# jenkinsm13/julia-spira

Measured on AMD Instinct MI355X. Metric: Msamples/sec at 1920x1080 spp=64 depth=8; fraction of HBM roofline, higher is better.
Workload: dtype f64

## Files before the change

julia-spira_amd/csrc/spira_device.h:

```cpp
#pragma once
#include <hip/hip_runtime.h>
#include <stdint.h>
#include <type_traits>
#include "spira_fastdiv.h"

namespace spira {

__device__ __forceinline__ float sqrt_rn(float x) { return __builtin_sqrtf(x); }
__device__ __forceinline__ double sqrt_rn(double x) { return __builtin_sqrt(x); }

constexpr int kBlock = 256;
#ifndef SPIRA_WAVES_F32
#define SPIRA_WAVES_F32 5
#endif
#ifndef SPIRA_WAVES_F64
#define SPIRA_WAVES_F64 4
#endif
#define SPIRA_WAVES_PER_SIMD(T) (sizeof(T) == 8 ? SPIRA_WAVES_F64 : SPIRA_WAVES_F32)
constexpr uint32_t kMaxTries = 64;

template <class T> struct Vec { T x, y, z; };

template <class T> __device__ __forceinline__ Vec<T> mk(T x, T y, T z) { Vec<T> r; r.x = x; r.y = y; r.z = z; return r; }
template <class T> __device__ __forceinline__ Vec<T> operator+(Vec<T> a, Vec<T> b) { return mk<T>(a.x + b.x, a.y + b.y, a.z + b.z); }
// ... 1143 lines not shown
        }
        wave_lds_sync();
#pragma unroll
        for (int r = 0; r < R; ++r) {
            const bool alive = pend[r].kind != kDead;
            const unsigned long long m = __ballot(alive);
            if (alive) {
                Vec<T> rnd = mk<T>(0, 0, 0);
                if (pend[r].kind != kMirror) { const Pack4<T> w = s_rnd[ent[r]]; rnd = mk<T>(w.x, w.y, w.z); }
                const Vec<T> nd = segment_back<T>(o[r], pend[r], rnd);
                const uint32_t dst = region + fill + __popcll(m & lt_mask);
                Pack4<T> A, B; Pack2<T> C;
                A.x = o[r].x; A.y = o[r].y; A.z = o[r].z; A.w = nd.x;
                B.x = nd.y; B.y = nd.z; B.z = beta[r].x; B.w = beta[r].y;
                C.x = beta[r].z; C.y = Bits<T>::from_u32(q[r]);
                a.qout.A[dst] = A; a.qout.B[dst] = B; a.qout.C[dst] = C;
            }
            fill += (uint32_t)__popcll(m);
        }
        wave_lds_sync();
    }
    for (int sft = 32; sft > 0; sft >>= 1) { n_rmw += __shfl_down(n_rmw, sft); n_seg += __shfl_down(n_seg, sft); n_store += __shfl_down(n_store, sft); }
    if (lane == 0) {
        if (scatter) a.cnt_out[wid] = fill;
        a.blk_stats[4 * wid] = n_seg;
        a.blk_stats[4 * wid + 1] = n_rmw;
        a.blk_stats[4 * wid + 2] = n_store;
        a.blk_stats[4 * wid + 3] = FIRST ? 0u : n_seg;
    }
}

template <class T> struct PathArgs {
    SceneGlobal<T> scene;
    RenderConst<T> rc;
    RayQueue<T> q[2];
    uint32_t *qref[2];
    uint2 *qkey[2];
    uint32_t cam_consts;
    Pack3<T> *L;
    uint32_t *blk_stats;
    uint32_t cap;
    uint32_t pass;
    uint32_t n_first;
    uint32_t dense_pct;
    Pack4<T> *mesh_list;
    uint32_t mesh_min_batch;
    uint32_t refill_free;
    uint32_t mesh_mode;
    uint32_t *mesh_count;
    uint32_t resume_k, resume_nw;
    uint32_t *redo;
    uint32_t redo_only;
    Stats *stats;
};

__device__ __forceinline__ float pack_qref(uint32_t q, uint32_t, float) { return __uint_as_float(q); }
__device__ __forceinline__ double pack_qref(uint32_t q, uint32_t ref, double) { return __longlong_as_double((long long)((unsigned long long)q | ((unsigned long long)ref << 32))); }
__device__ __forceinline__ uint32_t unpack_q(float w) { return __float_as_uint(w); }
__device__ __forceinline__ uint32_t unpack_q(double w) { return (uint32_t)(unsigned long long)__double_as_longlong(w); }
__device__ __forceinline__ uint32_t unpack_ref(double w) { return (uint32_t)((unsigned long long)__double_as_longlong(w) >> 32); }

#ifdef SPIRA_MESH_STATS
__device__ unsigned long long g_mesh_dbg[32];
#define MESH_STAT(...) __VA_ARGS__
#else
#define MESH_STAT(...)
#endif

#ifndef SPIRA_CARRY_KEY
#define SPIRA_CARRY_KEY 1
#endif
#ifndef SPIRA_WAVES_B_F32
#define SPIRA_WAVES_B_F32 4
#endif
#ifndef SPIRA_WAVES_B_F64
#define SPIRA_WAVES_B_F64 SPIRA_WAVES_F64
#endif
#ifndef SPIRA_WAVES_PATH_F32
#define SPIRA_WAVES_PATH_F32 6
#endif
template <class T, int R, bool BVH, bool EXT, bool SPEC, int MODE = 0, bool TRI = true>
__global__ __launch_bounds__(kBlock, MODE == 2 ? (sizeof(T) == 8 ? SPIRA_WAVES_B_F64 : SPIRA_WAVES_B_F32) : (sizeof(T) == 4 ? SPIRA_WAVES_PATH_F32 : SPIRA_WAVES_F64)) void k_path(const PathArgs<T> a) {
    extern __shared__ __attribute__((aligned(32))) unsigned char lds_raw[];
    constexpr uint32_t WPB = kBlock / 64, SUB = 64 * R;
    constexpr bool kRefArray = sizeof(T) == 4;
    constexpr bool kCarry = SPIRA_CARRY_KEY && !BVH && !EXT;
    constexpr uint32_t kStageShift = 25, kRefMask = (1u << kStageShift) - 1u;
    const uint32_t lane = threadIdx.x & 63, wave = threadIdx.x >> 6;
    const uint32_t NW = gridDim.x * WPB, wid = blockIdx.x * WPB + wave;
    const RenderConst<T> &rc = a.rc;
    using Pol = typename std::conditional<SPEC, SpecDiv, ExactDiv>::type;
    Pol pol;
    if (!SPEC && a.redo_only) {
        uint32_t any = 0;
        for (uint32_t w = 0; w < WPB; ++w) any |= a.redo[blockIdx.x * WPB + w];
        if (!any) return;
    }
    T *cam_lds = reinterpret_cast<T *>(lds_raw + scene_lds_bytes<T>(a.scene.n_spheres, a.scene.n_materials, a.scene.n_triangles) + WPB * SUB * sizeof(Pack4<T>));
    if (threadIdx.x < 12) {
        const Vec<T> *cv = threadIdx.x < 3 ? &rc.cam_origin : (threadIdx.x < 6 ? &rc.cam_llc : (threadIdx.x < 9 ? &rc.cam_hor : &rc.cam_ver));
        const uint32_t cc = threadIdx.x % 3;
        cam_lds[threadIdx.x] = cc == 0 ? cv->x : (cc == 1 ? cv->y : cv->z);
    }
    Pack4<T> *cam_sph = reinterpret_cast<Pack4<T> *>(reinterpret_cast<unsigned char *>(cam_lds) + 128);
    constexpr bool kCam = !EXT;
    if (kCam && MODE != 2 && a.cam_consts)
        for (uint32_t i = threadIdx.x; i < a.scene.n_spheres; i += blockDim.x) {
            const T *sp = a.scene.spheres5 + 5 * (size_t)i;
            const Vec<T> oc = rc.cam_origin - mk<T>(sp[0], sp[1], sp[2]);
            Pack4<T> k; k.x = oc.x; k.y = oc.y; k.z = oc.z; k.w = dot(oc, oc) - sp[3] * sp[3];
            cam_sph[i] = k;
        }
    const SceneLds<T> sc = stage_scene<T>(a.scene, lds_raw);
    const PixelDiv<T> pix_div = pixel_divisors<T>(rc);
    if (!SPEC && a.redo_only) {
        if (!a.redo[wid]) return;
        if (lane == 0) atomicAdd(&a.stats->redone_waves, 1ull);
    }
    Pack4<T> *s_rnd = reinterpret_cast<Pack4<T> *>(lds_raw + scene_lds_bytes<T>(a.scene.n_spheres, a.scene.n_materials, a.scene.n_triangles)) + wave * SUB;
    constexpr uint32_t mesh_mode = BVH ? (uint32_t)MODE : 0u;
    const uint32_t kseg = mesh_mode == 2u ? a.resume_k : 1u;
    if (mesh_mode == 2u && wid * kseg >= a.resume_nw) return;
    const uint32_t region = wid * kseg * a.cap;
    const unsigned long long lt_mask = (1ull << lane) - 1ull;
    const uint32_t ref_base = sc.n_spheres + sc.n_triangles;
    const bool mixed = mesh_mode != 0u || rc.max_depth <= 128u;
    const uint32_t dense_pct = mixed ? a.dense_pct : 0u;
    const bool defer = mesh_mode != 0u || (BVH && mixed && a.mesh_list != nullptr);
    Pack4<T> *mlist = a.mesh_list + 3 * (size_t)region;
    uint32_t n_rmw = 0, n_store = 0, n_seg = 0, n_enq = 0, n_park = 0;
    uint32_t n_wtrips = 0, n_ltrips = 0;
    uint32_t n_in = 0;
    const uint32_t n_sub_first = (a.n_first + SUB - 1) / SUB;

    auto park = [&](uint32_t slot_i, const Vec<T> o_, const Vec<T> d_, const Vec<T> beta_, T closest_, uint32_t q_, int prim_, uint32_t stage_hit) {
        Pack4<T> A, B, C;
        A.x = o_.x; A.y = o_.y; A.z = o_.z; A.w = d_.x;
        B.x = d_.y; B.y = d_.z; B.z = beta_.x; B.w = beta_.y;
        C.x = beta_.z; C.y = closest_; C.z = Bits<T>::from_u32(q_); C.w = Bits<T>::from_u32((uint32_t)(prim_ + 1) | (stage_hit << kStageShift));
        mlist[3 * (size_t)slot_i] = A; mlist[3 * (size_t)slot_i + 1] = B; mlist[3 * (size_t)slot_i + 2] = C;
    };
    uint32_t mfill = 0;
    constexpr int kMaxSeg = 16;
    uint32_t pfx[kMaxSeg + 1];
    bool segmented = false;
    {
        uint32_t cnt = 0;
        if (mesh_mode == 2u && lane < kseg && wid * kseg + lane < a.resume_nw) cnt = a.mesh_count[wid * kseg + lane];
        pfx[0] = 0;
#pragma unroll
        for (int j = 0; j < kMaxSeg; ++j) pfx[j + 1] = pfx[j] + (uint32_t)__builtin_amdgcn_readlane((int)cnt, j);
        if (mesh_mode == 2u) { mfill = pfx[kMaxSeg]; segmented = true; }
    }
    const uint32_t first_sub = mesh_mode == 1u ? (wid % a.resume_k) * (NW / a.resume_k) + wid / a.resume_k : wid;
    MESH_STAT(unsigned long long dbg_t0 = __builtin_readcyclecounter(); unsigned long long dbg_sess = 0, dbg_walk = 0; uint32_t dbg_ns = 0, dbg_ws = 0, dbg_ls = 0, dbg_rf = 0, dbg_rays = 0, dbg_rounds = 0, dbg_ws1 = 0, dbg_ls1 = 0, dbg_h[4] = {0, 0, 0, 0};)
    for (uint32_t round = 0; ; ++round) {
        MESH_STAT(++dbg_rounds;)
        const bool first = mesh_mode != 2u && round == 0;
        const RayQueue<T> qin = a.q[(round + 1) & 1], qout = a.q[round & 1];
        const uint32_t *rin = a.qref[(round + 1) & 1];
        uint32_t *rout = a.qref[round & 1];
        const uint2 *kin = a.qkey[(round + 1) & 1];
        uint2 *kout = a.qkey[round & 1];
        const uint32_t limit = first ? a.n_first : n_in;
        const uint32_t n_sub = first ? n_sub_first : (n_in + SUB - 1) / SUB;
        uint32_t fill = 0;
        for (uint32_t sub = first ? first_sub : 0u; sub < n_sub; sub += first ? NW : 1u) {
            Vec<T> o[R], beta[R];
            Pending<T> pend[R];
            ExtState<T> ex[R];
            uint32_t q[R], ent[R], stg[R], ref[R];
            uint32_t ka[R], kb[R];
            bool valid[R];
#pragma unroll
            for (int r = 0; r < R; ++r) {
                const uint32_t idx = sub * SUB + r * 64 + lane;
                valid[r] = false; stg[r] = round; ref[r] = 0; q[r] = 0; ka[r] = 0; kb[r] = 0;
                pend[r].kind = kDead; pend[r].rough = 0; pend[r].v = mk<T>(0, 0, 0);
                o[r] = mk<T>(0, 0, 0); beta[r] = mk<T>(1, 1, 1);
                bool parked = false; T park_t = 0; int park_prim = -1;
                if (idx < limit) {
                    if (first) {
                        uint32_t pixel, sample, pi, pj;
                        Vec<T> d;
                        q[r] = idx;
                        path_of<T>(rc, idx, a.pass, pi, pj, pixel, sample);
                        if (kCarry) { ka[r] = mix32(rc.sA + pixel) ^ (sample << 8); kb[r] = mix32(rc.sB ^ pixel) + (sample << 8); }
                        camera_ray_lds<T>(rc, cam_lds, pix_div, pi, pj, pixel, sample, o[r], d, pol);
                        if (EXT) { ex[r].flags = rc.flags; if (rc.flags & kExtSpectral) beta[r] = ext_wavelength<T>(sc, rc.sA, rc.sB, pixel, sample, ex[r]); }
                        T t; uint32_t slot = 0;
                        int prim;
                        if (defer) {
                            if (kCam && a.cam_consts) closest_hit_local<T, Pol, TRI, true>(sc, o[r], d, (T)0.001, t, prim, pol, cam_sph);
                            else closest_hit_local<T, Pol, TRI>(sc, o[r], d, (T)0.001, t, prim, pol);
                            parked = mesh_box_hit<T>(sc, o[r], d, t);
                        } else if (kCam && !BVH && a.cam_consts) { closest_hit_local<T, Pol, TRI, true>(sc, o[r], d, (T)0.001, t, prim, pol, cam_sph); }
                        else prim = closest_hit<T, BVH, Pol, TRI>(sc, o[r], d, (T)0.001, t, slot, pol);
                        ++n_seg;
                        if (parked) { park_t = t; park_prim = prim; pend[r].v = d; }
                        else if (prim < 0) {
                            const Vec<T> c = sky_term_x<T, EXT>(d, beta[r], &ex[r]);
                            Pack3<T> l; l.x = c.x; l.y = c.y; l.z = c.z;
                            a.L[idx] = l;
                            ++n_store;
                        } else {
                            valid[r] = true;
                            o[r] = o[r] + d * t;
                            ref[r] = (BVH && prim >= (int)ref_base) ? ref_base + slot : (uint32_t)prim;
                            pend[r].v = d;
                        }
                    } else {
                        const Pack4<T> A = qin.A[region + idx], B = qin.B[region + idx];
                        const Pack2<T> C = qin.C[region + idx];
                        o[r] = mk<T>(A.x, A.y, A.z);
                        pend[r].v = mk<T>(A.w, B.x, B.y);
                        beta[r] = mk<T>(B.z, B.w, C.x);
                        q[r] = unpack_q(C.y);
                        uint32_t w;
                        if constexpr (kRefArray) w = rin[region + idx]; else w = unpack_ref(C.y);
                        if (mixed) { stg[r] = w >> kStageShift; ref[r] = w & kRefMask; } else ref[r] = w;
                        if (kCarry) { const uint2 k = kin[region + idx]; ka[r] = k.x; kb[r] = k.y; }
                        valid[r] = true;
                    }
                }
                if (defer && first) {
                    const unsigned long long mp = __ballot(parked);
                    if (parked) park(mfill + __popcll(mp & lt_mask), o[r], pend[r].v, beta[r], park_t, q[r], park_prim, 0u);
                    mfill += (uint32_t)__popcll(mp); n_park += (uint32_t)__popcll(mp);
                }
            }
            while (true) {
                uint32_t n_list = 0, n_valid = 0;
#pragma unroll
                for (int r = 0; r < R; ++r) {
                    bool want = false;
                    RngKey key;
                    const Vec<T> d = pend[r].v;
                    pend[r].kind = kDead;
                    if (valid[r]) {
                        uint32_t pixel = 0, sample = 0, pi, pj;
                        const bool scatter = stg[r] + 1 < rc.max_depth;
                        int prim = (int)ref[r]; uint32_t slot = 0;
                        if (BVH && ref[r] >= ref_base) { prim = (int)ref_base; slot = ref[r] - ref_base; }
                        const uint32_t qi = q[r] & 0x7FFFFFFFu;
                        const bool has_l = (q[r] >> 31) != 0;
                        if (EXT) {
                            path_of<T>(rc, qi, a.pass, pi, pj, pixel, sample);
                            ex[r].flags = rc.flags;
                            if (rc.flags & kExtSpectral) (void)ext_wavelength<T>(sc, rc.sA, rc.sB, pixel, sample, ex[r]);
                        }
                        Vec<T> contrib;
                        const bool has_contrib = shade_hit<T, BVH, EXT, Pol, TRI>(sc, o[r], d, prim, slot, beta[r], scatter, contrib, pend[r], &ex[r], pol);
                        if (has_contrib) {
                            Pack3<T> l; l.x = contrib.x; l.y = contrib.y; l.z = contrib.z;
                            if (has_l) { const Pack3<T> l0 = a.L[qi]; l.x = l0.x + contrib.x; l.y = l0.y + contrib.y; l.z = l0.z + contrib.z; ++n_rmw; }
                            else ++n_store;
// ... 293 lines not shown
                finished = false;
                const unsigned long long mf = __ballot(!walking);
                const uint32_t take = min((uint32_t)__popcll(mf), mfill - next);
                if (!walking && (uint32_t)__popcll(mf & lt_mask) < take) {
                    const uint32_t e = next + (uint32_t)__popcll(mf & lt_mask);
                    const Pack4<T> *ent = mlist + 3 * (size_t)e;
                    if (segmented) {
                        uint32_t seg = 0, off = e;
#pragma unroll
                        for (int j = 1; j < kMaxSeg; ++j) if (e >= pfx[j]) { seg = (uint32_t)j; off = e - pfx[j]; }
                        ent = a.mesh_list + 3 * ((size_t)(wid * kseg + seg) * a.cap + off);
                    }
                    const Pack4<T> A = ent[0], B = ent[1], C = ent[2];
                    o_ = mk<T>(A.x, A.y, A.z); d_ = mk<T>(A.w, B.x, B.y); beta_ = mk<T>(B.z, B.w, C.x);
                    closest = C.y;
                    q_ = Bits<T>::to_u32(C.z);
                    const uint32_t pw = Bits<T>::to_u32(C.w);
                    prim = (int)(pw & kRefMask) - 1;
                    stage_hit = pw >> kStageShift;
                    slot = 0;
                    T t0;
                    if (bvh8_enter<T>(sc, o_, d_, closest, ry, t0)) { bvh8_begin<T>(wk, ry, t0, (T)0.001, sc.bvh_root[2].w); walking = true; }
                    else finished = true;
                }
                next += take;
                if (!__any(walking)) { if (__any(finished)) continue; break; }
                const bool more = next < mfill;
                MESH_STAT(++dbg_rf; const unsigned long long dbg_w0 = __builtin_readcyclecounter();)
                uint32_t n_now = (uint32_t)__popcll(__ballot(walking));
                while (true) {
                    ++n_wtrips; n_ltrips += n_now;
                    MESH_STAT(++dbg_ws; { const uint32_t nl = (uint32_t)__popcll(__ballot(walking)); dbg_ls += nl; if (segmented) { ++dbg_ws1; dbg_ls1 += nl; } ++dbg_h[nl <= 8 ? 0 : (nl <= 24 ? 1 : (nl <= 48 ? 2 : 3))]; })
                    if (walking && !bvh8_step<T, kLdsStack>(sc, wk, ry, o_, d_, (T)0.001, (int)ref_base, closest, prim, slot, lstack, stack, lane)) { walking = false; finished = true; }
                    const uint32_t n_walk = (uint32_t)__popcll(__ballot(walking));
                    n_now = n_walk;
                    if (n_walk == 0 || (more && 64u - n_walk >= a.refill_free)) break;
                }

                MESH_STAT(dbg_walk += __builtin_readcyclecounter() - dbg_w0;)
            }
            }
            mfill = 0;
            segmented = false;
            MESH_STAT(dbg_sess += __builtin_readcyclecounter() - dbg_s0;)
        }
        n_in = fill;
        n_enq += fill;
        if (n_in == 0 && (mfill == 0 || mesh_mode == 1u)) break;
        __builtin_amdgcn_fence(__ATOMIC_RELEASE, "workgroup");
        __builtin_amdgcn_fence(__ATOMIC_ACQUIRE, "workgroup");
    }
    for (int sft = 32; sft > 0; sft >>= 1) { n_rmw += __shfl_down(n_rmw, sft); n_seg += __shfl_down(n_seg, sft); n_store += __shfl_down(n_store, sft); }
    const bool again = SPEC && __any(outside_window<T>(pol));
    MESH_STAT(if (lane == 0) { unsigned long long *g = g_mesh_dbg + (mesh_mode == 2u ? 16 : 0);
                               atomicAdd(&g[0], __builtin_readcyclecounter() - dbg_t0); atomicAdd(&g[1], dbg_sess); atomicAdd(&g[2], (unsigned long long)dbg_ns);
                               atomicAdd(&g[3], (unsigned long long)dbg_ws); atomicAdd(&g[4], (unsigned long long)dbg_ls); atomicAdd(&g[5], (unsigned long long)dbg_rf);
                               atomicAdd(&g[6], (unsigned long long)dbg_rays); atomicAdd(&g[7], (unsigned long long)dbg_rounds); atomicAdd(&g[9], dbg_walk); atomicAdd(&g[10], 1ull); atomicAdd(&g[11], (unsigned long long)dbg_ws1); atomicAdd(&g[12], (unsigned long long)dbg_ls1);
                               atomicAdd(&g[8], (unsigned long long)dbg_h[0]); atomicAdd(&g[13], (unsigned long long)dbg_h[1]); atomicAdd(&g[14], (unsigned long long)dbg_h[2]); atomicAdd(&g[15], (unsigned long long)dbg_h[3]); })
    if (lane == 0) {
        if (mesh_mode == 2u) {
            const uint32_t row = 4 * wid * kseg;
            a.blk_stats[row] += n_seg; a.blk_stats[row + 1] += n_rmw; a.blk_stats[row + 2] += n_store; a.blk_stats[row + 3] += n_enq;
        } else {
            a.blk_stats[4 * wid] = n_seg;
            a.blk_stats[4 * wid + 1] = n_rmw;
            a.blk_stats[4 * wid + 2] = n_store;
            a.blk_stats[4 * wid + 3] = n_enq;
            if (mesh_mode == 1u) a.mesh_count[wid] = mfill;
        }
        if (SPEC) a.redo[wid] = again ? 1u : 0u;
        if (BVH && n_park && !again && !(SPEC && a.redo_only == 2u)) atomicAdd(&a.stats->rays_parked, (unsigned long long)n_park);
        if (BVH && mesh_mode != 1u && n_wtrips && !again && !(SPEC && a.redo_only == 2u)) { atomicAdd(&a.stats->mesh_wave_trips, (unsigned long long)n_wtrips); atomicAdd(&a.stats->mesh_lane_trips, (unsigned long long)n_ltrips); }
    }
}

template <class T, bool BVH, bool EXT>
__global__ __launch_bounds__(kBlock) void k_mega(const BounceArgs<T> a) {
    extern __shared__ __attribute__((aligned(32))) unsigned char lds_raw[];
    const SceneLds<T> sc = stage_scene<T>(a.scene, lds_raw);
    const RenderConst<T> &rc = a.rc;
    unsigned long long nseg = 0;
    const uint32_t stride = gridDim.x * kBlock;
    uint32_t idx = blockIdx.x * kBlock + threadIdx.x;
    bool fresh = true;
    uint32_t pixel = 0, sample = 0, b = 0;
    Vec<T> o = mk<T>(0, 0, 0), d = mk<T>(0, 0, 1), beta = mk<T>(1, 1, 1), Lacc = mk<T>(0, 0, 0);
    ExtState<T> ex; ex.flags = rc.flags; ex.bR = 0; ex.bG = 0; ex.bB = 0;
    while (idx < a.n_first) {
        if (fresh) {
            uint32_t pi, pj;
            path_of<T>(rc, idx, a.pass, pi, pj, pixel, sample);
            camera_ray<T>(rc, pi, pj, pixel, sample, o, d);
            beta = mk<T>(1, 1, 1); Lacc = mk<T>(0, 0, 0); b = 0;
            if (EXT && (rc.flags & kExtSpectral)) beta = ext_wavelength<T>(sc, rc.sA, rc.sB, pixel, sample, ex);
            fresh = false;
        }
        Vec<T> contrib; T t_hit;
        SegInfo si = trace_segment<T, BVH, EXT>(sc, rc, o, d, beta, pixel, sample, b, b + 1 < rc.max_depth, contrib, t_hit, &ex);
        ++nseg;
        if (b == 0) { if (si.has_contrib) Lacc = contrib; }
        else if (si.has_contrib) Lacc = Lacc + contrib;
        ++b;
        if (!si.alive || b == rc.max_depth) {
            Pack3<T> l; l.x = Lacc.x; l.y = Lacc.y; l.z = Lacc.z;
            a.L[idx] = l;
            idx += stride;
// ... 529 lines not shown
                }
            }
            n_in = fill;
            n_enq += fill;
            __builtin_amdgcn_fence(__ATOMIC_RELEASE, "workgroup");
            __builtin_amdgcn_fence(__ATOMIC_ACQUIRE, "workgroup");
            if (n_in == 0) break;
        }
    }
    for (int sft = 32; sft > 0; sft >>= 1) { n_seg += __shfl_down(n_seg, sft); n_rmw += __shfl_down(n_rmw, sft); n_store += __shfl_down(n_store, sft); }
    const bool again = SPEC && (a.redo_only == 2 || __any(outside_window<T>(pol)));
    if (lane == 0) {
        a.blk_stats[4 * wid] = n_seg;
        a.blk_stats[4 * wid + 1] = n_rmw;
        a.blk_stats[4 * wid + 2] = n_store;
        a.blk_stats[4 * wid + 3] = n_enq;
        if (SPEC) a.redo[wid] = again ? 1u : 0u;
    }
}

static __global__ void k_fold_stats(const uint32_t *blk_stats, uint32_t n_rows, Stats *stats) {
    unsigned long long seg = 0, enq = 0, rmw = 0, sto = 0;
    for (uint32_t i = threadIdx.x; i < n_rows; i += blockDim.x) { seg += blk_stats[4 * i]; rmw += blk_stats[4 * i + 1]; sto += blk_stats[4 * i + 2]; enq += blk_stats[4 * i + 3]; }
    for (int sft = 32; sft > 0; sft >>= 1) { seg += __shfl_down(seg, sft); enq += __shfl_down(enq, sft); rmw += __shfl_down(rmw, sft); sto += __shfl_down(sto, sft); }
    if (threadIdx.x == 0) { stats->segments += seg; stats->rays_enqueued += enq; stats->radiance_rmw += rmw; stats->radiance_store += sto; }
}

template <class T, int SEM>
__global__ __launch_bounds__(64) void k_trace_variant(const BounceArgs<T> a, const uint32_t *ijs, uint32_t n_paths, int *prims, T *ts,
                                                      T *dirs, T *radiance) {
    extern __shared__ __attribute__((aligned(32))) unsigned char lds_raw[];
    const SceneLds<T> sc = stage_scene<T>(a.scene, lds_raw);
    const RenderConst<T> &rc = a.rc;
    uint32_t p = blockIdx.x * blockDim.x + threadIdx.x;
    if (p >= n_paths) return;
    uint32_t i = ijs[3 * p], j = ijs[3 * p + 1], sample = ijs[3 * p + 2];
    int *pr = prims + (size_t)p * rc.max_depth;
    T *pt = ts + (size_t)p * rc.max_depth, *pd = dirs + 3 * (size_t)p * rc.max_depth;
    Vec<T> c = mk<T>(0, 0, 0);
    uint32_t nseg = 0;
    if (SEM == 1) {
        nseg = path_cpu<T>(sc, rc, i, j, sample, c, pr, pt, pd);
    } else {
        uint32_t st = metal_state0(rc.sA, rc.sB, (j - 1) * rc.width + (i - 1));
        for (uint32_t s = 0; s <= sample; ++s) nseg = path_metal<T>(sc, rc, i - 1, j - 1, st, c, pr, pt, pd);
    }
    for (uint32_t b = nseg; b < rc.max_depth; ++b) pr[b] = -2;
    radiance[3 * p] = c.x; radiance[3 * p + 1] = c.y; radiance[3 * p + 2] = c.z;
}

template <class T>
__global__ __launch_bounds__(kBlock) void k_resolve(Pack4<T> *accum, const Pack3<T> *L, uint32_t tile_pixels, uint32_t k_eff, int first_pass,
                                                    const uint32_t *blk_stats, uint32_t n_rows, Stats *stats) {
    for (uint32_t p = blockIdx.x * kBlock + threadIdx.x; p < tile_pixels; p += gridDim.x * kBlock) {
        Pack4<T> acc;
        if (first_pass) { acc.x = 0; acc.y = 0; acc.z = 0; acc.w = 0; } else acc = accum[p];
        uint32_t s = 0;
        for (; s + 8 <= k_eff; s += 8) {
            Pack3<T> l[8];
#pragma unroll
            for (int k = 0; k < 8; ++k) l[k] = L[(size_t)(s + k) * tile_pixels + p];
#pragma unroll
            for (int k = 0; k < 8; ++k) { acc.x = acc.x + l[k].x; acc.y = acc.y + l[k].y; acc.z = acc.z + l[k].z; }
        }
        for (; s < k_eff; ++s) {
            const Pack3<T> l = L[(size_t)s * tile_pixels + p];
            acc.x = acc.x + l.x; acc.y = acc.y + l.y; acc.z = acc.z + l.z;
        }
        accum[p] = acc;
    }
    if (blockIdx.x == 0 && blk_stats) {
        __shared__ unsigned long long red[4];
        if (threadIdx.x < 4) red[threadIdx.x] = 0;
        __syncthreads();
        unsigned long long seg = 0, enq = 0, rmw = 0, sto = 0;
        for (uint32_t i = threadIdx.x; i < n_rows; i += kBlock) {
            seg += blk_stats[4 * i];
            rmw += blk_stats[4 * i + 1];
            sto += blk_stats[4 * i + 2];
            enq += blk_stats[4 * i + 3];
        }
        for (int sft = 32; sft > 0; sft >>= 1) { seg += __shfl_down(seg, sft); enq += __shfl_down(enq, sft); rmw += __shfl_down(rmw, sft); sto += __shfl_down(sto, sft); }
        if ((threadIdx.x & 63) == 0) { atomicAdd(&red[0], seg); atomicAdd(&red[1], enq); atomicAdd(&red[2], rmw); atomicAdd(&red[3], sto); }
        __syncthreads();
        if (threadIdx.x == 0) { stats->segments += red[0]; stats->rays_enqueued += red[1]; stats->radiance_rmw += red[2]; stats->radiance_store += red[3]; }
    }
}

template <class T> __host__ __device__ inline T aces1(T x) {
    const T a = (T)2.51, b = (T)0.03, c = (T)2.43, d = (T)0.59, e = (T)0.14;
    T v = (x * (a * x + b)) / (x * (c * x + d) + e);
    return v < 0 ? (T)0 : (v > 1 ? (T)1 : v);
}
__host__ __device__ inline float sqrt_any(float x) { return __builtin_sqrtf(x); }
__host__ __device__ inline double sqrt_any(double x) { return __builtin_sqrt(x); }
template <class T> struct HybridPx { Vec<T> d, o, pt, n; };
template <class T> struct HybridArgs {
    SceneGlobal<T> scene;
    RenderConst<T> rc;
    T *state;
    uint32_t *mat;
    uint32_t *rng;
    Pack4<T> *accum;
    uint32_t *flags;
    Stats *stats;
    uint32_t sample;
    uint32_t phase;
};
__device__ __forceinline__ uint32_t xorshift32_step(uint32_t s) { s ^= s << 13; s ^= s >> 17; s ^= s << 5; return s; }
template <class T> __device__ __forceinline__ T xs_uniform(uint32_t s) { return (T)(float)((double)s / 4294967295.0); }
template <class T> __device__ __forceinline__ T aces_sqrt(T x) {
    const T a = (T)2.51f, b = (T)0.03f, c = (T)2.43f, d = (T)0.59f, e = (T)0.14f;
    T r = (x * (a * x + b)) / (x * (c * x + d) + e);
    r = r < (T)0 ? (T)0 : (r > (T)1 ? (T)1 : r);
    return sqrt_rn(r);
}
template <class T>
__global__ __launch_bounds__(kBlock) void k_hybrid(const HybridArgs<T> a) {
    extern __shared__ __attribute__((aligned(32))) unsigned char lds_raw[];
    const RenderConst<T> &rc = a.rc;
    const uint32_t P = rc.width * rc.height, D = rc.max_depth;
    uint32_t *fl = a.flags + (size_t)(a.sample - 1) * (D + 1);
    if (a.phase > 0 && fl[a.phase] == 0) return;
// ... 148 lines not shown
```

julia-spira_amd/csrc/spira_hip.hip:

```cpp
#include <hip/hip_runtime.h>
#include <sys/mman.h>
#include <rccl/rccl.h>
#include <dlfcn.h>

#include <algorithm>
#include <atomic>
#include <chrono>
#include <cmath>
#include <cstdio>
#include <cstdlib>
#include <cstring>
#include <condition_variable>
#include <mutex>
#include <new>
#include <string>
#include <thread>
#include <vector>

#include "../../include/spira_hip.h"
#include "../../include/spira_spd.h"
#include "spira_device.h"
#include "spira_bvh.h"
#include "spira_validate.h"

// ... 525 lines not shown
    return 0;
}

struct PathPlan {
    uint64_t waves = 0;
    uint64_t packets = 0;
    uint64_t batch = 0;
    bool queues = false;
    bool mesh = false;
    bool two_pass = false;
    bool spec = false;
};
template <class T>
int ensure_path_plan(Ctx &c, const PathPlan &pl) {
    using P4 = spira::Pack4<T>;
    using P2 = spira::Pack2<T>;
    if (pl.queues)
        for (int i = 0; i < 2; ++i) {
            if (int rc = c.qA[i].ensure(pl.packets * sizeof(P4))) return rc;
            if (int rc = c.qB[i].ensure(pl.packets * sizeof(P4))) return rc;
            if (int rc = c.qC[i].ensure(pl.packets * sizeof(P2))) return rc;
            if (sizeof(T) == 4) { if (int rc = c.qR[i].ensure(pl.packets * sizeof(uint32_t))) return rc; }
            if (!pl.mesh) { if (int rc = c.qK[i].ensure(pl.packets * sizeof(uint2))) return rc; }
        }
    if (pl.mesh) { if (int rc = c.mesh_list.ensure(3 * pl.packets * sizeof(P4))) return rc; }
    if (pl.two_pass) { if (int rc = c.mesh_count.ensure(pl.waves * sizeof(uint32_t))) return rc; }
    if (pl.spec) { if (int rc = c.redo.ensure(pl.waves * sizeof(uint32_t))) return rc; }
    if (int rc = c.blkstats.ensure(pl.waves * 4 * sizeof(uint32_t))) return rc;
    if (int rc = c.L.ensure(pl.batch * sizeof(spira::Pack3<T>))) return rc;
    return c.stats.ensure(sizeof(spira::Stats));
}
template <class T>
int verify_path_args(const Ctx &c, const spira::PathArgs<T> &a, uint32_t first_launch_blocks) {
    using P4 = spira::Pack4<T>;
    using P2 = spira::Pack2<T>;
    const uint64_t nw = (uint64_t)first_launch_blocks * (spira::kBlock / 64), n = nw * a.cap;
    auto covers = [](const DevBuf &b, const void *ptr, uint64_t bytes) { return ptr == b.p && b.p != nullptr && b.cap >= bytes; };
    const char *bad = nullptr;
    const bool mesh = a.scene.n_bvh_tris != 0;
    if ((uint64_t)a.n_first > n) bad = "the pass does not fit its queue regions";
    if (a.rc.max_depth > 1 || mesh)
        for (int i = 0; i < 2 && !bad; ++i) {
            if (!covers(c.qA[i], a.q[i].A, n * sizeof(P4)) || !covers(c.qB[i], a.q[i].B, n * sizeof(P4)) || !covers(c.qC[i], a.q[i].C, n * sizeof(P2))) bad = "hit queues";
            else if (sizeof(T) == 4 && !covers(c.qR[i], a.qref[i], n * sizeof(uint32_t))) bad = "hit reference arrays";
            else if (!mesh && !covers(c.qK[i], a.qkey[i], n * sizeof(uint2))) bad = "carried RNG keys";
        }
    if (!bad && a.mesh_list && !covers(c.mesh_list, a.mesh_list, 3 * n * sizeof(P4))) bad = "mesh lists";
    if (!bad && a.mesh_mode != 0 && (!a.mesh_list || !covers(c.mesh_count, a.mesh_count, nw * sizeof(uint32_t)) || a.resume_k == 0 || a.resume_k > 16 || nw % a.resume_k != 0 || a.resume_nw != nw))
        bad = "parked-ray counts of a two-launch mesh pass";
    if (!bad && a.redo && !covers(c.redo, a.redo, nw * sizeof(uint32_t))) bad = "redo flags";
    if (!bad && !covers(c.blkstats, a.blk_stats, nw * 4 * sizeof(uint32_t))) bad = "per-wave statistics";
    if (!bad && !covers(c.L, a.L, (uint64_t)a.n_first * sizeof(spira::Pack3<T>))) bad = "per-path radiance";
    if (!bad && !covers(c.stats, a.stats, sizeof(spira::Stats))) bad = "counters";
    if (bad) return fail(SPIRA_E_LIMIT, std::string("internal: a workspace is smaller than the launch needs (") + bad + ")");
    return 0;
}

template <class T>
int render_impl(const spira_scene *h, const T *spheres5, const T *materials8, const T *triangles10, const T *camera12, const spira_params *p,
                T *out_hdr, T *out_img, bool out_on_device, void *user_stream,
                bool progressive = false, uint32_t sample0 = 0, uint32_t *rng_states = nullptr, const SlabCtl *slab = nullptr) {
    uint32_t rows = 0;
    const bool cont = slab && slab->index > 0;
    if (!p) return fail(SPIRA_E_INVALID, "params is NULL");
    tl_lds_optin = hipSuccess;
    Lap lap("render");
    if (h) { if (int rc = check_handle<T>(h)) return rc; }
    else if (!cont) { if (int rc = validate_scene<T>(spheres5, materials8, triangles10, p->n_spheres, p->n_materials, triangles10 ? p->n_triangles : 0)) return rc; }
    if (int rc = validate_params(camera12, p, h ? h->store.nt : (triangles10 ? p->n_triangles : 0), &rows)) return rc;
    lap("validate");
    if (!out_hdr && !out_img) return fail(SPIRA_E_INVALID, "both outputs are NULL");
    if (progressive && (uint64_t)sample0 + p->spp > SPIRA_MAX_SPP) return fail(SPIRA_E_LIMIT, "sample0 + spp exceeds 2^24");
    if (progressive && (p->flags & SPIRA_SEM_MASK) == SPIRA_SEM_HYBRID) return fail(SPIRA_E_UNSUPPORTED, "SPIRA_SEM_HYBRID has no accumulate entry (its image is a mean of tone-mapped samples)");
    if (progressive && (p->flags & SPIRA_SEM_MASK) == SPIRA_SEM_METAL && sample0 > 0 && !rng_states)
        return fail(SPIRA_E_INVALID, "SPIRA_SEM_METAL with sample0 > 0 needs rng_states (the LCG states the previous call left); "
                                     "without them every call would replay the samples of the first");
    Ctx *cp = nullptr;
    if (int rc = get_ctx(&cp)) return rc;
    Ctx &c = *cp;
    std::lock_guard<std::recursive_mutex> lock(c.mu);
    hipStream_t st = out_on_device ? (hipStream_t)user_stream : c.stream;
    if (int rc = order_after_previous(c, st)) return rc;
    lap("context");

    const uint32_t W = p->width;
    const uint64_t tile_pixels = (uint64_t)rows * W;
    uint32_t target = p->batch_rays ? p->batch_rays : env_u32("SPIRA_BATCH_RAYS", 160u << 20);
    uint64_t slots64 = std::max<uint64_t>(1, target / tile_pixels);
    slots64 = std::min<uint64_t>(slots64, p->spp);
    slots64 = (p->spp + (p->spp + slots64 - 1) / slots64 - 1) / ((p->spp + slots64 - 1) / slots64);
    if (slots64 * tile_pixels > 0x7FFFFFFFull) return fail(SPIRA_E_LIMIT, "tile too large: rows*width must be < 2^31");
    const uint32_t slots = (uint32_t)slots64;
    const uint64_t batch = slots64 * tile_pixels;
    const uint32_t sem = p->flags & SPIRA_SEM_MASK;
    const bool mega = (p->flags & SPIRA_KERNEL_MASK) == SPIRA_KERNEL_MEGA || sem != SPIRA_SEM_A;
    const bool metal_wavefront = sem == SPIRA_SEM_METAL && (p->flags & SPIRA_KERNEL_MASK) == SPIRA_KERNEL_WAVEFRONT;
    uint64_t metal_launches = 0;
    const bool per_bounce = !mega && (p->flags & SPIRA_KERNEL_MASK) == SPIRA_KERNEL_BOUNCE;
    const bool persistent = !mega && !per_bounce;
    const bool profile = ((p->flags & SPIRA_FLAG_PROFILE) != 0 && per_bounce) || persistent;
    int R = (int)env_u32("SPIRA_R", 2);
    if (R != 1 && R != 2) R = 2;
    if (p->flags & (SPIRA_EXT_DIELECTRIC | SPIRA_EXT_SPECTRAL)) R = 2;

    const uint32_t nt_scene = h ? h->store.nt : (triangles10 ? p->n_triangles : 0);
    const bool mesh_two_pass = persistent && nt_scene > SPIRA_LDS_TRIANGLES && p->max_depth <= 128 && env_u32("SPIRA_DEFER_MESH", 1) && env_u32("SPIRA_MESH_TWO_PASS", 1);
    const uint32_t blocks_per_cu = !persistent ? 16 : ((nt_scene > SPIRA_LDS_TRIANGLES && !mesh_two_pass) ? 4 : 32);
    const uint32_t max_blocks = (uint32_t)c.num_cus * env_u32("SPIRA_BLOCKS_PER_CU", blocks_per_cu);
    const uint32_t wpb = spira::kBlock / 64;
    const uint32_t sub = 64 * R;
    auto geometry = [&](uint64_t n_first, uint32_t &G, uint32_t &cap) {
        const uint64_t n_sub = (n_first + sub - 1) / sub;
        G = (uint32_t)std::min<uint64_t>((n_sub + wpb - 1) / wpb, max_blocks);
        const uint64_t nw = (uint64_t)G * wpb;
        cap = (uint32_t)(((n_sub + nw - 1) / nw) * sub);
    };
    uint32_t G_max = 0, cap_max = 0;
    geometry(batch, G_max, cap_max);
    const uint64_t q_rays = (uint64_t)cap_max * G_max * wpb;
    if (q_rays > 0xFFFFFFFFull) return fail(SPIRA_E_LIMIT, "pass too large");

    using P4 = spira::Pack4<T>;
    using P2 = spira::Pack2<T>;
    const bool mesh_scene = nt_scene > SPIRA_LDS_TRIANGLES;
    const bool defer_mesh = persistent && mesh_scene && p->max_depth <= 128 && env_u32("SPIRA_DEFER_MESH", 1) != 0;
    PathPlan plan;
    plan.waves = (uint64_t)G_max * wpb; plan.packets = q_rays; plan.batch = batch;
    plan.queues = !mega && (p->max_depth > 1 || (persistent && mesh_scene));
    plan.mesh = defer_mesh; plan.two_pass = defer_mesh && mesh_two_pass; plan.spec = persistent && env_u32("SPIRA_SPEC_DIV", 1) != 0;
    if (persistent) { if (int rc = ensure_path_plan<T>(c, plan)) return rc; }
    else {
        if (plan.queues)
            for (int i = 0; i < 2; ++i) {
                if (int rc = c.qA[i].ensure(q_rays * sizeof(P4))) return rc;
                if (int rc = c.qB[i].ensure(q_rays * sizeof(P4))) return rc;
                if (int rc = c.qC[i].ensure(q_rays * sizeof(P2))) return rc;
            }
        if (sem != SPIRA_SEM_HYBRID) { if (int rc = c.L.ensure(batch * sizeof(spira::Pack3<T>))) return rc; }
        if (per_bounce) { if (int rc = c.counts.ensure((size_t)(p->max_depth + 2) * G_max * wpb * sizeof(uint32_t))) return rc; }
        if (int rc = c.blkstats.ensure((size_t)(per_bounce ? p->max_depth + 1 : 1) * G_max * wpb * 4 * sizeof(uint32_t))) return rc;
        if (int rc = c.stats.ensure(sizeof(spira::Stats))) return rc;
    }
    if (int rc = c.accum.ensure(tile_pixels * sizeof(P4))) return rc;

    lap("workspaces");
    spira::BounceArgs<T> a{};
    if (int rc = acquire_scene<T>(c, st, h, spheres5, materials8, triangles10, p, a.scene, cont)) return rc;
    if (int rc = attach_spd<T>(c, st, p, a.scene)) return rc;
    lap("scene");
    const bool scene_moderate = h ? h->store.moderate : c.scene.moderate;
    fill_const<T>(a.rc, camera12, p, rows, slots);
    if (!fastdiv_selfcheck(a.rc.tile_pixels, (uint32_t)batch) || !fastdiv_selfcheck(a.rc.width, a.rc.tile_pixels) ||
        !fastdiv_selfcheck(a.rc.stripe_h ? a.rc.stripe_h : 1, rows))
        return fail(SPIRA_E_LIMIT, "internal: fast division self-check failed");
    a.L = (spira::Pack3<T> *)c.L.p;
    a.stats = (spira::Stats *)c.stats.p;

    const size_t lds = spira::scene_lds_bytes<T>(a.scene.n_spheres, a.scene.n_materials, a.scene.n_triangles);
    const uint32_t n_pass = (p->spp + slots - 1) / slots;

    T *d_hdr = out_hdr, *d_img = out_img;
    if (!out_on_device) {
        size_t plane3 = 3 * tile_pixels * sizeof(T);
        if (int rc = c.out_tmp.ensure(2 * plane3)) return rc;
// ... 129 lines not shown
            uint32_t G = 0, stat_rows = 0;
            if (sem == SPIRA_SEM_CPU) {
                uint32_t blocks = std::min<uint32_t>((n_first + spira::kBlock - 1) / spira::kBlock, max_blocks);
                int spec = (int)env_u32("SPIRA_SPEC_DIV", 1);
                if (spec == 1 && !(scene_moderate && spira::camera_scale_moderate<T>(camera12))) spec = 0;
                if (spec == 3) spec = 1;
                if (spec) {
                    if (int rc = c.redo.ensure((size_t)max_blocks * wpb * sizeof(uint32_t))) return rc;
                    uint32_t *redo = (uint32_t *)c.redo.p;
                    launch_lds(spira::k_variant_cpu<T, true>, dim3(blocks), dim3(spira::kBlock), lds, st, a, redo, spec == 2 ? 2 : 0);
                    launch_lds(spira::k_variant_cpu<T, false>, dim3(blocks), dim3(spira::kBlock), lds, st, a, redo, 1);
                    launches += 2;
                } else {
                    launch_lds(spira::k_variant_cpu<T, false>, dim3(blocks), dim3(spira::kBlock), lds, st, a, (uint32_t *)nullptr, 0);
                    ++launches;
                }
            } else if (mega) {
                uint32_t blocks = std::min<uint32_t>((n_first + spira::kBlock - 1) / spira::kBlock, max_blocks);
                const bool ext = (p->flags & (SPIRA_EXT_DIELECTRIC | SPIRA_EXT_SPECTRAL)) != 0;
                if (a.scene.n_bvh_tris) { if (ext) launch_lds(spira::k_mega<T, true, true>, dim3(blocks), dim3(spira::kBlock), lds, st, a); else launch_lds(spira::k_mega<T, true, false>, dim3(blocks), dim3(spira::kBlock), lds, st, a); }
                else { if (ext) launch_lds(spira::k_mega<T, false, true>, dim3(blocks), dim3(spira::kBlock), lds, st, a); else launch_lds(spira::k_mega<T, false, false>, dim3(blocks), dim3(spira::kBlock), lds, st, a); }
                ++launches;
            } else if (persistent) {
                spira::PathArgs<T> pa{};
                pa.scene = a.scene; pa.rc = a.rc; pa.L = a.L; pa.pass = pass; pa.n_first = n_first;
                pa.dense_pct = std::min<uint32_t>(env_u32("SPIRA_DENSE_PCT", 70), 100);
                pa.mesh_list = plan.mesh ? (P4 *)c.mesh_list.p : nullptr;
                geometry(n_first, G, pa.cap);
                stat_rows = G * wpb;
                for (int i = 0; i < 2; ++i) {
                    pa.q[i] = {(P4 *)c.qA[i].p, (P4 *)c.qB[i].p, (P2 *)c.qC[i].p};
                    pa.qref[i] = (uint32_t *)c.qR[i].p;
                    pa.qkey[i] = (uint2 *)c.qK[i].p;
                }
                pa.blk_stats = (uint32_t *)c.blkstats.p;
                pa.stats = (spira::Stats *)c.stats.p;
                int spec = (int)env_u32("SPIRA_SPEC_DIV", 1);
                if (spec == 1 && !(scene_moderate && spira::camera_scale_moderate<T>(camera12))) spec = 0;
                if (spec == 3) spec = 1;
                if (spec) pa.redo = (uint32_t *)c.redo.p;
                pa.mesh_mode = 0; pa.mesh_count = nullptr; pa.resume_k = 1; pa.resume_nw = 0;
                pa.mesh_min_batch = std::max<uint32_t>(1, env_u32("SPIRA_MESH_MIN_BATCH", 128));
                pa.refill_free = std::min<uint32_t>(64, std::max<uint32_t>(1, env_u32("SPIRA_MESH_REFILL", 16)));
                size_t lds_a = lds + (size_t)wpb * sub * sizeof(P4) + 128;
                pa.cam_consts = (env_u32("SPIRA_CAM_CONSTS", 1) && a.scene.n_spheres && lds_a + (size_t)a.scene.n_spheres * sizeof(P4) <= (size_t)160 * 1024) ? 1u : 0u;
                if (pa.cam_consts) lds_a += (size_t)a.scene.n_spheres * sizeof(P4);
                if (plan.two_pass) {
                    pa.mesh_mode = 1; pa.mesh_count = (uint32_t *)c.mesh_count.p;
                    const uint32_t nw = G * wpb, fat = std::max<uint32_t>(1, (uint32_t)c.num_cus * env_u32("SPIRA_MESH_FAT_WAVES_PER_CU", 16));
                    uint32_t k = 16;
                    while (k > 1 && (nw % k != 0 || nw / k < fat)) k >>= 1;
                    pa.resume_k = k; pa.resume_nw = nw;
                }
                if (int rc = verify_path_args<T>(c, pa, G)) return rc;
                HIP_TRY(hipEventRecord(c.ev_pool[c.ev_used++], st));
                if (int rc = launch_path<T>(R, dim3(G), lds_a, st, pa, spec)) return rc;
                if (int rc = lds_optin_failed()) return rc;
                launches += (spec && R == 2) ? 2 : 1;
                if (pa.mesh_mode == 1) {
                    if (c.ev_mid.size() <= c.ev_mid_used) {
                        hipEvent_t e;
                        HIP_TRY(hipEventCreate(&e));
                        c.ev_mid.push_back(e); c.ev_mid_end.push_back(0);
                    }
                    HIP_TRY(hipEventRecord(c.ev_mid[c.ev_mid_used], st));
                    c.ev_mid_end[c.ev_mid_used++] = c.ev_used;
                    spira::PathArgs<T> pb = pa;
                    pb.mesh_mode = 2; pb.n_first = 0;
                    const uint32_t nwb = pa.resume_nw / pa.resume_k;
                    launch_path_resume_entry<T>(R, dim3((nwb + wpb - 1) / wpb), lds_a, st, pb);
                    if (int rc = lds_optin_failed()) return rc;
                    ++launches;
                }
                HIP_TRY(hipEventRecord(c.ev_pool[c.ev_used++], st));
            } else {
                geometry(n_first, G, a.cap);
                stat_rows = p->max_depth * G * wpb;
                const size_t nw = (size_t)G * wpb;
                for (uint32_t b = 0; b < p->max_depth; ++b) {
                    a.bounce = b;
                    int qi = b & 1;
                    a.qout = {(P4 *)c.qA[qi].p, (P4 *)c.qB[qi].p, (P2 *)c.qC[qi].p};
                    a.qin = {(P4 *)c.qA[qi ^ 1].p, (P4 *)c.qB[qi ^ 1].p, (P2 *)c.qC[qi ^ 1].p};
                    a.cnt_in = (const uint32_t *)c.counts.p + (size_t)b * nw;
                    a.cnt_out = (uint32_t *)c.counts.p + (size_t)(b + 1) * nw;
                    a.blk_stats = (uint32_t *)c.blkstats.p + (size_t)b * nw * 4;
                    if (profile) HIP_TRY(hipEventRecord(c.ev_pool[c.ev_used++], st));
                    const size_t lds_b = lds + (size_t)wpb * sub * sizeof(P4);
                    if (b == 0) launch_bounce<T, true>(R, dim3(G), lds_b, st, a);
                    else launch_bounce<T, false>(R, dim3(G), lds_b, st, a);
                    if (int rc = lds_optin_failed()) return rc;
                    if (profile) HIP_TRY(hipEventRecord(c.ev_pool[c.ev_used++], st));
                    ++launches;
                }
            }
            uint32_t rblocks = std::min<uint32_t>((uint32_t)((tile_pixels + spira::kBlock - 1) / spira::kBlock), max_blocks);
            hipLaunchKernelGGL((spira::k_resolve<T>), dim3(rblocks), dim3(spira::kBlock), 0, st, (P4 *)c.accum.p, (const spira::Pack3<T> *)c.L.p,
                               (uint32_t)tile_pixels, k_eff, (pass == 0 && !progressive) ? 1 : 0, mega ? (const uint32_t *)nullptr : (const uint32_t *)c.blkstats.p,
                               stat_rows, (spira::Stats *)c.stats.p);
            ++launches;
        }
    }
    {
        uint32_t fblocks = std::min<uint32_t>((uint32_t)((tile_pixels + spira::kBlock - 1) / spira::kBlock), max_blocks);
        if (progressive)
            hipLaunchKernelGGL((spira::k_finalize<T>), dim3(fblocks), dim3(spira::kBlock), 0, st, (const P4 *)c.accum.p, (uint32_t)tile_pixels,
                               1u, (uint32_t)SPIRA_POST_NONE, d_hdr, (T *)nullptr);
        else
            hipLaunchKernelGGL((spira::k_finalize<T>), dim3(fblocks), dim3(spira::kBlock), 0, st, (const P4 *)c.accum.p, (uint32_t)tile_pixels,
                               p->spp, sem == SPIRA_SEM_HYBRID ? (uint32_t)SPIRA_POST_NONE : (p->flags & SPIRA_POST_MASK), d_hdr, d_img);
        ++launches;
    }
    if (progressive && rng_states && !out_on_device)
        HIP_TRY(hipMemcpyAsync(rng_states, d_rng, tile_pixels * sizeof(uint32_t), hipMemcpyDeviceToHost, st));
    if (int rc = lds_optin_failed()) return rc;
    HIP_TRY(hipGetLastError());
    HIP_TRY(hipEventRecord(c.ev_stop, st));
    HIP_TRY(hipMemcpyAsync(c.h_stats, c.stats.p, sizeof(spira::Stats), hipMemcpyDeviceToHost, st));
    lap("enqueue");

    if (!cont) c.last = spira_counters{};
    c.last.samples += (uint64_t)p->spp * tile_pixels;
    c.last.passes += p->max_depth ? n_pass : 0;
    c.last.launches += launches;
    c.last.bounce_launches += metal_launches ? metal_launches : ((mega || !p->max_depth) ? 0 : (uint64_t)n_pass * (persistent ? 1 : p->max_depth));
    c.last_valid = true;
    c.last_pending = true;
    c.last_stream = st;

    if (!out_on_device) {
        void *const dst[2] = {out_hdr, out_img};
        const void *const src[2] = {d_hdr, d_img};
        if (int rc = copy_out(c, st, dst, src, 3 * tile_pixels * sizeof(T))) return rc;
    }
    if (int rc = mark_done(c, st)) return rc;
    if (!out_on_device) HIP_TRY(hipStreamSynchronize(st));
    lap("copy_out+sync");
    return 0;
}

template <class T>
int render_entry_plain(const spira_scene *h, const T *spheres5, const T *materials8, const T *triangles10, const T *camera12, const spira_params *p,
                       T *out_hdr, T *out_img, bool out_on_device, void *user_stream, bool progressive = false, uint32_t sample0 = 0, uint32_t *rng_states = nullptr,
                       const SlabCtl *slab = nullptr) {
#ifdef SPIRA_TU_MAIN
    if constexpr (sizeof(T) == 4)
        return spira_tu::render_impl_f32(h, spheres5, materials8, triangles10, camera12, p, out_hdr, out_img, out_on_device, user_stream, progressive, sample0, rng_states, slab);
    else
// ... 726 lines not shown
```

Baseline: 24980.

## Fuse per-pixel radiance resolve into persistent path kernel with pixel-owning waves

In the f64 sphere-only persistent path, each wave now owns a fixed set of pixels and traces all k_eff samples for them. It then sums the per-sample radiance into the accumulator itself, so the separate k_resolve launch is skipped. Pixels are interleaved in runs of four across waves, the grid is sized from the pixel count, and per-wave stats are flushed with atomics instead of through the blkstats reduction. This removes a kernel launch and a full re-read of L from HBM. In exchange the first-round work distribution changes from a global strided split to a per-wave fixed one, which risks load imbalance and different occupancy.

```diff
diff --git a/julia-spira_amd/csrc/spira_device.h b/julia-spira_amd/csrc/spira_device.h
--- a/julia-spira_amd/csrc/spira_device.h
+++ b/julia-spira_amd/csrc/spira_device.h
@@ -1219,7 +1219,39 @@
     uint32_t *redo;
     uint32_t redo_only;
     Stats *stats;
+    Pack4<T> *accum;
+    FastDiv fd_keff;
+    uint32_t k_eff;
+    uint32_t accum_first;
 };
+
+#ifndef SPIRA_RESOLVE_RUN
+#define SPIRA_RESOLVE_RUN 4
+#endif
+__device__ __forceinline__ uint32_t owned_pixel(uint32_t w, uint32_t nw, uint32_t l) {
+    constexpr uint32_t kRun = SPIRA_RESOLVE_RUN;
+    static_assert(64 % kRun == 0, "a run length divides the wave");
+    return ((l / kRun) * nw + w) * kRun + l % kRun;
+}
+
+template <class T>
+__device__ __forceinline__ void resolve_pixel(Pack4<T> *accum, const Pack3<T> *L, uint32_t tile_pixels, uint32_t k_eff, bool first_pass, uint32_t p) {
+    Pack4<T> acc;
+    if (first_pass) { acc.x = 0; acc.y = 0; acc.z = 0; acc.w = 0; } else acc = accum[p];
+    uint32_t s = 0;
+    for (; s + 8 <= k_eff; s += 8) {
+        Pack3<T> l[8];
+#pragma unroll
+        for (int k = 0; k < 8; ++k) l[k] = L[(size_t)(s + k) * tile_pixels + p];
+#pragma unroll
+        for (int k = 0; k < 8; ++k) { acc.x = acc.x + l[k].x; acc.y = acc.y + l[k].y; acc.z = acc.z + l[k].z; }
+    }
+    for (; s < k_eff; ++s) {
+        const Pack3<T> l = L[(size_t)s * tile_pixels + p];
+        acc.x = acc.x + l.x; acc.y = acc.y + l.y; acc.z = acc.z + l.z;
+    }
+    accum[p] = acc;
+}
 
 __device__ __forceinline__ float pack_qref(uint32_t q, uint32_t, float) { return __uint_as_float(q); }
 __device__ __forceinline__ double pack_qref(uint32_t q, uint32_t ref, double) { return __longlong_as_double((long long)((unsigned long long)q | ((unsigned long long)ref << 32))); }
@@ -1298,7 +1330,9 @@
     uint32_t n_rmw = 0, n_store = 0, n_seg = 0, n_enq = 0, n_park = 0;
     uint32_t n_wtrips = 0, n_ltrips = 0;
     uint32_t n_in = 0;
-    const uint32_t n_sub_first = (a.n_first + SUB - 1) / SUB;
+    const bool own = !BVH && !EXT && !TRI && sizeof(T) == 8 && a.accum != nullptr;
+    const uint32_t n_own = own ? 64u * a.k_eff : 0u;
+    const uint32_t n_sub_first = own ? (n_own + SUB - 1) / SUB : (a.n_first + SUB - 1) / SUB;
 
     auto park = [&](uint32_t slot_i, const Vec<T> o_, const Vec<T> d_, const Vec<T> beta_, T closest_, uint32_t q_, int prim_, uint32_t stage_hit) {
         Pack4<T> A, B, C;
@@ -1319,7 +1353,8 @@
         for (int j = 0; j < kMaxSeg; ++j) pfx[j + 1] = pfx[j] + (uint32_t)__builtin_amdgcn_readlane((int)cnt, j);
         if (mesh_mode == 2u) { mfill = pfx[kMaxSeg]; segmented = true; }
     }
-    const uint32_t first_sub = mesh_mode == 1u ? (wid % a.resume_k) * (NW / a.resume_k) + wid / a.resume_k : wid;
+    const uint32_t first_sub = own ? 0u : (mesh_mode == 1u ? (wid % a.resume_k) * (NW / a.resume_k) + wid / a.resume_k : wid);
+    const uint32_t sub_step = own ? 1u : NW;
     MESH_STAT(unsigned long long dbg_t0 = __builtin_readcyclecounter(); unsigned long long dbg_sess = 0, dbg_walk = 0; uint32_t dbg_ns = 0, dbg_ws = 0, dbg_ls = 0, dbg_rf = 0, dbg_rays = 0, dbg_rounds = 0, dbg_ws1 = 0, dbg_ls1 = 0, dbg_h[4] = {0, 0, 0, 0};)
     for (uint32_t round = 0; ; ++round) {
         MESH_STAT(++dbg_rounds;)
@@ -1329,10 +1364,10 @@
         uint32_t *rout = a.qref[round & 1];
         const uint2 *kin = a.qkey[(round + 1) & 1];
         uint2 *kout = a.qkey[round & 1];
-        const uint32_t limit = first ? a.n_first : n_in;
+        const uint32_t limit = first ? (own ? n_own : a.n_first) : n_in;
         const uint32_t n_sub = first ? n_sub_first : (n_in + SUB - 1) / SUB;
         uint32_t fill = 0;
-        for (uint32_t sub = first ? first_sub : 0u; sub < n_sub; sub += first ? NW : 1u) {
+        for (uint32_t sub = first ? first_sub : 0u; sub < n_sub; sub += first ? sub_step : 1u) {
             Vec<T> o[R], beta[R];
             Pending<T> pend[R];
             ExtState<T> ex[R];
@@ -1346,12 +1381,20 @@
                 pend[r].kind = kDead; pend[r].rough = 0; pend[r].v = mk<T>(0, 0, 0);
                 o[r] = mk<T>(0, 0, 0); beta[r] = mk<T>(1, 1, 1);
                 bool parked = false; T park_t = 0; int park_prim = -1;
-                if (idx < limit) {
+                uint32_t qf = idx;
+                bool in = idx < limit;
+                if (own && first) {
+                    const uint32_t t = idx / SPIRA_RESOLVE_RUN, run = fastdiv(t, a.fd_keff);
+                    const uint32_t px = owned_pixel(wid, NW, run * SPIRA_RESOLVE_RUN + idx % SPIRA_RESOLVE_RUN);
+                    qf = (t - run * a.k_eff) * rc.tile_pixels + px;
+                    in = in && px < rc.tile_pixels;
+                }
+                if (in) {
                     if (first) {
                         uint32_t pixel, sample, pi, pj;
                         Vec<T> d;
-                        q[r] = idx;
-                        path_of<T>(rc, idx, a.pass, pi, pj, pixel, sample);
+                        q[r] = qf;
+                        path_of<T>(rc, qf, a.pass, pi, pj, pixel, sample);
                         if (kCarry) { ka[r] = mix32(rc.sA + pixel) ^ (sample << 8); kb[r] = mix32(rc.sB ^ pixel) + (sample << 8); }
                         camera_ray_lds<T>(rc, cam_lds, pix_div, pi, pj, pixel, sample, o[r], d, pol);
                         if (EXT) { ex[r].flags = rc.flags; if (rc.flags & kExtSpectral) beta[r] = ext_wavelength<T>(sc, rc.sA, rc.sB, pixel, sample, ex[r]); }
@@ -1368,7 +1411,7 @@
                         else if (prim < 0) {
                             const Vec<T> c = sky_term_x<T, EXT>(d, beta[r], &ex[r]);
                             Pack3<T> l; l.x = c.x; l.y = c.y; l.z = c.z;
-                            a.L[idx] = l;
+                            a.L[qf] = l;
                             ++n_store;
                         } else {
                             valid[r] = true;
@@ -1768,6 +1811,17 @@
     }
     for (int sft = 32; sft > 0; sft >>= 1) { n_rmw += __shfl_down(n_rmw, sft); n_seg += __shfl_down(n_seg, sft); n_store += __shfl_down(n_store, sft); }
     const bool again = SPEC && __any(outside_window<T>(pol));
+    if (own && !again && !(SPEC && a.redo_only == 2u)) {
+        __builtin_amdgcn_fence(__ATOMIC_RELEASE, "workgroup");
+        __builtin_amdgcn_fence(__ATOMIC_ACQUIRE, "workgroup");
+        const uint32_t px = owned_pixel(wid, NW, lane);
+        if (px < rc.tile_pixels) resolve_pixel<T>(a.accum, a.L, rc.tile_pixels, a.k_eff, a.accum_first != 0, px);
+        const uint32_t seg = __shfl(n_seg, 0), rmw = __shfl(n_rmw, 0), sto = __shfl(n_store, 0);
+        if (lane < 4) {
+            unsigned long long *f = lane == 0 ? &a.stats->segments : (lane == 1 ? &a.stats->rays_enqueued : (lane == 2 ? &a.stats->radiance_rmw : &a.stats->radiance_store));
+            atomicAdd(f, (unsigned long long)(lane == 0 ? seg : (lane == 1 ? n_enq : (lane == 2 ? rmw : sto))));
+        }
+    }
     MESH_STAT(if (lane == 0) { unsigned long long *g = g_mesh_dbg + (mesh_mode == 2u ? 16 : 0);
                                atomicAdd(&g[0], __builtin_readcyclecounter() - dbg_t0); atomicAdd(&g[1], dbg_sess); atomicAdd(&g[2], (unsigned long long)dbg_ns);
                                atomicAdd(&g[3], (unsigned long long)dbg_ws); atomicAdd(&g[4], (unsigned long long)dbg_ls); atomicAdd(&g[5], (unsigned long long)dbg_rf);
@@ -2403,23 +2457,8 @@
 template <class T>
 __global__ __launch_bounds__(kBlock) void k_resolve(Pack4<T> *accum, const Pack3<T> *L, uint32_t tile_pixels, uint32_t k_eff, int first_pass,
                                                     const uint32_t *blk_stats, uint32_t n_rows, Stats *stats) {
-    for (uint32_t p = blockIdx.x * kBlock + threadIdx.x; p < tile_pixels; p += gridDim.x * kBlock) {
-        Pack4<T> acc;
-        if (first_pass) { acc.x = 0; acc.y = 0; acc.z = 0; acc.w = 0; } else acc = accum[p];
-        uint32_t s = 0;
-        for (; s + 8 <= k_eff; s += 8) {
-            Pack3<T> l[8];
-#pragma unroll
-            for (int k = 0; k < 8; ++k) l[k] = L[(size_t)(s + k) * tile_pixels + p];
-#pragma unroll
-            for (int k = 0; k < 8; ++k) { acc.x = acc.x + l[k].x; acc.y = acc.y + l[k].y; acc.z = acc.z + l[k].z; }
-        }
-        for (; s < k_eff; ++s) {
-            const Pack3<T> l = L[(size_t)s * tile_pixels + p];
-            acc.x = acc.x + l.x; acc.y = acc.y + l.y; acc.z = acc.z + l.z;
-        }
-        accum[p] = acc;
-    }
+    for (uint32_t p = blockIdx.x * kBlock + threadIdx.x; p < tile_pixels; p += gridDim.x * kBlock)
+        resolve_pixel<T>(accum, L, tile_pixels, k_eff, first_pass != 0, p);
     if (blockIdx.x == 0 && blk_stats) {
         __shared__ unsigned long long red[4];
         if (threadIdx.x < 4) red[threadIdx.x] = 0;
diff --git a/julia-spira_amd/csrc/spira_hip.hip b/julia-spira_amd/csrc/spira_hip.hip
--- a/julia-spira_amd/csrc/spira_hip.hip
+++ b/julia-spira_amd/csrc/spira_hip.hip
@@ -601,6 +601,12 @@
     if (!bad && !covers(c.blkstats, a.blk_stats, nw * 4 * sizeof(uint32_t))) bad = "per-wave statistics";
     if (!bad && !covers(c.L, a.L, (uint64_t)a.n_first * sizeof(spira::Pack3<T>))) bad = "per-path radiance";
     if (!bad && !covers(c.stats, a.stats, sizeof(spira::Stats))) bad = "counters";
+    if (!bad && a.accum) {
+        const uint64_t tp = a.rc.tile_pixels;
+        if (!covers(c.accum, a.accum, tp * sizeof(spira::Pack4<T>)) || sizeof(T) != 8 || a.scene.n_triangles || mesh || (a.rc.flags & (SPIRA_EXT_DIELECTRIC | SPIRA_EXT_SPECTRAL)) ||
+            a.k_eff == 0 || a.k_eff > 64 || (uint64_t)a.k_eff * tp != a.n_first || 64 * nw < tp || a.cap < 64ull * a.k_eff)
+            bad = "pixel-owning pass";
+    }
     if (bad) return fail(SPIRA_E_LIMIT, std::string("internal: a workspace is smaller than the launch needs (") + bad + ")");
     return 0;
 }
@@ -658,7 +664,15 @@
     const uint32_t max_blocks = (uint32_t)c.num_cus * env_u32("SPIRA_BLOCKS_PER_CU", blocks_per_cu);
     const uint32_t wpb = spira::kBlock / 64;
     const uint32_t sub = 64 * R;
+    const bool fused = persistent && sizeof(T) == 8 && R == 2 && nt_scene == 0 && (p->flags & (SPIRA_EXT_DIELECTRIC | SPIRA_EXT_SPECTRAL)) == 0 &&
+                       slots <= 64 && env_u32("SPIRA_FUSED_RESOLVE", 1) != 0;
     auto geometry = [&](uint64_t n_first, uint32_t &G, uint32_t &cap) {
+        if (fused) {
+            const uint64_t k = n_first / tile_pixels;
+            G = (uint32_t)((tile_pixels + 64 * wpb - 1) / (64 * wpb));
+            cap = (uint32_t)((64 * k + sub - 1) / sub * sub);
+            return;
+        }
         const uint64_t n_sub = (n_first + sub - 1) / sub;
         G = (uint32_t)std::min<uint64_t>((n_sub + wpb - 1) / wpb, max_blocks);
         const uint64_t nw = (uint64_t)G * wpb;
@@ -894,6 +908,10 @@
                     while (k > 1 && (nw % k != 0 || nw / k < fat)) k >>= 1;
                     pa.resume_k = k; pa.resume_nw = nw;
                 }
+                if (fused) {
+                    pa.accum = (P4 *)c.accum.p; pa.k_eff = k_eff; pa.fd_keff = spira::fastdiv_make(k_eff);
+                    pa.accum_first = (pass == 0 && !progressive) ? 1u : 0u;
+                }
                 if (int rc = verify_path_args<T>(c, pa, G)) return rc;
                 HIP_TRY(hipEventRecord(c.ev_pool[c.ev_used++], st));
                 if (int rc = launch_path<T>(R, dim3(G), lds_a, st, pa, spec)) return rc;
@@ -936,6 +954,7 @@
                     ++launches;
                 }
             }
+            if (fused) continue;
             uint32_t rblocks = std::min<uint32_t>((uint32_t)((tile_pixels + spira::kBlock - 1) / spira::kBlock), max_blocks);
             hipLaunchKernelGGL((spira::k_resolve<T>), dim3(rblocks), dim3(spira::kBlock), 0, st, (P4 *)c.accum.p, (const spira::Pack3<T> *)c.L.p,
                                (uint32_t)tile_pixels, k_eff, (pass == 0 && !progressive) ? 1 : 0, mega ? (const uint32_t *)nullptr : (const uint32_t *)c.blkstats.p,
```

After: 26260, median of 6. +5.1%, better.
